# Consensys/gnark

Hardware: AMD Instinct MI355X
Metric: G1 MSM throughput, BN254, 2^24 scalar-muls on one GPU (Groth16 proofs/s at 2^24 constraints in 'groth16') (higher is better)
Workload: dtype u64 Montgomery limbs in memory; 29/28-bit limbs, v_mad_u64_u32 (32x32+64) in registers

## Files before the change

gnark_amd/csrc/msm.hip.h:

```cpp
#pragma once
#include <cstring>
#include <hipcub/hipcub.hpp>
#include <rocprim/device/device_radix_sort.hpp>

#include <string>

#include "common.hip.h"
#include "field29.hip.h"

namespace ga {

constexpr int GA_ACC29_MINW = 4;
#ifndef GA_ACC29_FP2_MINW
#define GA_ACC29_FP2_MINW 2
#endif
constexpr uint32_t MSM_SIGN = 0x80000000u;
constexpr int MSM_HOT_TASKS = 16;
constexpr uint32_t MSM_VHOT_TASKS = 512;
constexpr uint32_t MSM_VHOT_SPLIT = 64;
constexpr int MSM_GROUP = 32;

typedef rocprim::radix_sort_config<rocprim::default_config, rocprim::default_config,
                                   rocprim::radix_sort_onesweep_config<rocprim::kernel_config<1024, 21>, rocprim::kernel_config<1024, 21>, 11,
                                                                       rocprim::block_radix_rank_algorithm::match>>
// ... 661 lines not shown
__device__ __forceinline__ uint32_t msm_multi_dest(const MsmTables& mt, uint32_t dest) {
    return dest < mt.nb ? dest + blockIdx.y * mt.nb : dest + (mt.k - 1) * mt.nb + blockIdx.y * mt.max_tasks;
}

#ifdef GA_ACC29_NUM_VGPR
#define GA_ACC29_VGPR_ATTR __attribute__((amdgpu_waves_per_eu(GA_ACC29_NUM_VGPR, GA_ACC29_NUM_VGPR)))
#else
#define GA_ACC29_VGPR_ATTR
#endif
template <class F, bool COMPLETE>
__global__ void __launch_bounds__(Table29<F>::THREADS, Table29<F>::MIN_WAVES) GA_ACC29_VGPR_ATTR
msm_accumulate29_kernel(const MsmTables mt, const uint32_t* __restrict__ vals,
                        const uint32_t* __restrict__ task_start, const uint32_t* __restrict__ task_qkey_sorted,
                        const uint32_t* __restrict__ task_key_by_tid, const uint32_t* __restrict__ task_perm, uint32_t max_tasks, uint32_t seg,
                        const uint32_t* __restrict__ task_dest, XYZZ<F>* __restrict__ sums, uint32_t* __restrict__ redo_list,
                        uint32_t* __restrict__ redo_count) {
    constexpr int NW = Lazy<F>::NW;
    __shared__ uint32_t lds[4 * NW * Table29<F>::THREADS];
    uint32_t t = blockIdx.x * blockDim.x + threadIdx.x;
    if (t >= max_tasks) return;
    if (task_qkey_sorted[t] == 0xFFFFFFFFu) return;
    const uint32_t tid = task_perm[t];
    const uint32_t key = task_key_by_tid[tid];
    const uint32_t start = task_start[tid];
    LdsAcc29<F> A(lds + threadIdx.x);
    const bool have = accumulate_task29<F, COMPLETE>(A, mt.t[blockIdx.y], vals, start, start + (seg - key));
    if (!store_task29<F>(A, have, &sums[msm_multi_dest(mt, task_dest[tid])]))
        redo_list[(uint64_t)blockIdx.y * (mt.max_tasks + 2) + atomicAdd(redo_count + 2 * blockIdx.y, 1u)] = tid;
}

template <class F>
__global__ void __launch_bounds__(Table29<F>::THREADS, Table29<F>::MIN_WAVES)
msm_accumulate29_retry_kernel(const MsmTables mt, const uint32_t* __restrict__ vals,
                              const uint32_t* __restrict__ task_start, const uint32_t* __restrict__ task_key_by_tid, uint32_t seg,
                              const uint32_t* __restrict__ redo_list, const uint32_t* __restrict__ redo_count,
                              const uint32_t* __restrict__ task_dest, XYZZ<F>* __restrict__ sums, uint32_t* __restrict__ redo2_list,
                              uint32_t* __restrict__ redo2_count) {
    constexpr int NW = Lazy<F>::NW;
    __shared__ uint32_t lds[4 * NW * Table29<F>::THREADS];
    redo_list += (uint64_t)blockIdx.y * (mt.max_tasks + 2);
    redo2_list += (uint64_t)blockIdx.y * (mt.max_tasks + 2);
    const uint32_t nredo = redo_count[2 * blockIdx.y];
    LdsAcc29<F> A(lds + threadIdx.x);
    for (uint32_t r = blockIdx.x * blockDim.x + threadIdx.x; r < nredo; r += gridDim.x * blockDim.x) {
        const uint32_t tid = redo_list[r];
        const uint32_t start = task_start[tid];
        const bool have = accumulate_task29<F, true>(A, mt.t[blockIdx.y], vals, start, start + (seg - task_key_by_tid[tid]));
        if (!store_task29<F>(A, have, &sums[msm_multi_dest(mt, task_dest[tid])])) redo2_list[atomicAdd(redo2_count + 2 * blockIdx.y, 1u)] = tid;
    }
}

template <class F>
__global__ void __launch_bounds__(64)
msm_accumulate29_redo_kernel(const MsmTables mt, const uint32_t* __restrict__ vals,
                             const uint32_t* __restrict__ task_start, const uint32_t* __restrict__ task_key_by_tid,
                             uint32_t seg, const uint32_t* __restrict__ redo_list, const uint32_t* __restrict__ redo_count,
                             const uint32_t* __restrict__ task_dest, XYZZ<F>* __restrict__ sums) {
    typedef typename Lazy<F>::T T;
    redo_list += (uint64_t)blockIdx.y * (mt.max_tasks + 2);
    const uint32_t nredo = redo_count[2 * blockIdx.y];
    const uint32_t* __restrict__ table = mt.t[blockIdx.y];
    for (uint32_t r = blockIdx.x * blockDim.x + threadIdx.x; r < nredo; r += gridDim.x * blockDim.x) {
        const uint32_t tid = redo_list[r];
        const uint32_t start = task_start[tid];
        const uint32_t end = start + (seg - task_key_by_tid[tid]);
        XYZZ<F> acc = xyzz_inf<F>();
        for (uint32_t p = start; p < end; p++) {
            const uint32_t v = vals[p];
            T qx, qy;
            load_point29<F>(table, v & ~MSM_SIGN, qx, qy);
            Affine<F> q{Lazy<F>::to_mem(qx), Lazy<F>::to_mem(qy)};
            if (v & MSM_SIGN) q.y = neg(q.y);
            acc = madd(acc, q);
        }
        store_pod(&sums[msm_multi_dest(mt, task_dest[tid])], acc);
    }
}

template <class F> struct BaseFieldOf;
template <class Pp> struct BaseFieldOf<Fe<Pp>> { typedef Pp P; static constexpr bool IS_FP = true; };
template <class Pp> struct BaseFieldOf<Fe2<Pp>> { typedef Pp P; static constexpr bool IS_FP = false; };


template <class F>
__device__ __forceinline__ XYZZ<F> wave_tree_sum(XYZZ<F> acc, XYZZ<F>* sh) {
    const uint32_t lane = threadIdx.x;
    for (uint32_t stride = 32; stride >= 1; stride >>= 1) {
        sh[lane] = acc;
        __syncthreads();
        if (lane < stride) acc = add(acc, sh[lane + stride]);
        __syncthreads();
    }
    return acc;
}


template <class F>
__global__ void __launch_bounds__(64)
msm_reduce_groups_kernel(const XYZZ<F>* __restrict__ bsum, uint32_t half, uint32_t m, uint32_t groups_per_win,
                         uint32_t total_groups, XYZZ<F>* __restrict__ gsum) {
    uint32_t gid = blockIdx.x * blockDim.x + threadIdx.x;
    if (gid >= total_groups) return;
    uint32_t w = gid / groups_per_win, g = gid % groups_per_win;
    const XYZZ<F>* B = bsum + (uint64_t)w * half + (uint64_t)g * m;
    XYZZ<F> running = xyzz_inf<F>(), local = xyzz_inf<F>();
    for (int j = (int)m - 1; j >= 0; j--) {
        running = add(running, load_pod<XYZZ<F>>(&B[j]));
        local = add(local, running);
    }
    uint32_t base = g * m;
    if (base != 0) {
        XYZZ<F> r = xyzz_inf<F>();
        int top = 31 - __clz(base);
        for (int bit = top; bit >= 0; bit--) {
            r = dbl(r);
            if ((base >> bit) & 1) r = add(r, running);
        }
        local = add(local, r);
    }
    store_pod(&gsum[gid], local);
}

template <class F>
struct Lazy4 {
    typename Lazy<F>::T x, y, zz, zzz;
};
template <class F>
__device__ __forceinline__ Lazy4<F> lazy4_from_mem(const XYZZ<F>& p) {
    return {Lazy<F>::from_mem(p.x), Lazy<F>::from_mem(p.y), Lazy<F>::from_mem(p.zz), Lazy<F>::from_mem(p.zzz)};
}
template <class F>
__device__ __forceinline__ void add29(Lazy4<F>& a, const Lazy4<F>& b) {
    typedef typename Lazy<F>::T T;
    typedef typename Lazy<F>::Params P;
    constexpr int KMS = Lazy<F>::FP2 ? P::FP2Z_K : 8;
    T U1 = f29_mul(a.x, b.zz);
    T U2 = f29_mul(b.x, a.zz);
    T S1 = f29_mul(a.y, b.zzz);
    T S2 = f29_mul(b.y, a.zzz);
    T Pp = f29_sub<4>(U2, U1);
    T R = f29_sub<4>(S2, S1);
    T PP = f29_sqr(Pp);
    T PPP = f29_mul(Pp, PP);
    T Q = f29_mul(U1, PP);
    T X3 = f29_sub<4>(f29_sqr(R), f29_add(PPP, f29_add(Q, Q)));
    if constexpr (Lazy<F>::FP2) X3 = f29_partial_reduce(X3);
    a.y = f29_mul_sub<KMS>(R, f29_sub<8>(Q, X3), S1, PPP);
    a.x = X3;
    a.zz = f29_mul(f29_mul(a.zz, b.zz), PP);
    a.zzz = f29_mul(f29_mul(a.zzz, b.zzz), PPP);
}

template <class F>
__global__ void __launch_bounds__(64)
msm_reduce_groups29_kernel(const XYZZ<F>* __restrict__ bsum, uint32_t half, uint32_t m, uint32_t groups_per_win,
                           uint32_t total_groups, XYZZ<F>* __restrict__ lsum, XYZZ<F>* __restrict__ rsum,
                           uint32_t* __restrict__ redo_list, uint32_t* __restrict__ redo_count) {
    uint32_t gid = blockIdx.x * blockDim.x + threadIdx.x;
    if (gid >= total_groups) return;
    uint32_t w = gid / groups_per_win, g = gid % groups_per_win;
    const XYZZ<F>* B = bsum + (uint64_t)w * half + (uint64_t)g * m;
    Lazy4<F> running, local;
    bool r_inf = true, l_inf = true;
    for (int j = (int)m - 1; j >= 0; j--) {
        XYZZ<F> b = load_pod<XYZZ<F>>(&B[j]);
        if (!is_inf(b)) {
            Lazy4<F> lb = lazy4_from_mem<F>(b);
            if (r_inf) {
                running = lb;
                r_inf = false;
            } else {
                add29<F>(running, lb);
            }
        }
        if (!r_inf) {
            if (l_inf) {
                local = running;
                l_inf = false;
            } else {
                add29<F>(local, running);
            }
        }
    }
    XYZZ<F> lo = xyzz_inf<F>(), ro = xyzz_inf<F>();
    bool bad = false;
    if (!r_inf) {
        ro.zz = Lazy<F>::to_mem(running.zz);
        lo.zz = Lazy<F>::to_mem(local.zz);
        bad = is_zero(ro.zz) | is_zero(lo.zz);
        ro.x = Lazy<F>::to_mem(running.x);
        ro.y = Lazy<F>::to_mem(running.y);
        ro.zzz = Lazy<F>::to_mem(running.zzz);
        lo.x = Lazy<F>::to_mem(local.x);
        lo.y = Lazy<F>::to_mem(local.y);
        lo.zzz = Lazy<F>::to_mem(local.zzz);
    }
    if (bad) {
        redo_list[atomicAdd(redo_count, 1u)] = gid;
        return;
    }
    store_pod(&lsum[gid], lo);
    store_pod(&rsum[gid], ro);
}

template <class F>
__global__ void __launch_bounds__(64)
msm_reduce_groups_redo_kernel(const XYZZ<F>* __restrict__ bsum, uint32_t half, uint32_t m, uint32_t groups_per_win,
                              const uint32_t* __restrict__ redo_list, const uint32_t* __restrict__ redo_count,
                              XYZZ<F>* __restrict__ lsum, XYZZ<F>* __restrict__ rsum) {
    const uint32_t nredo = *redo_count;
    for (uint32_t r = blockIdx.x * blockDim.x + threadIdx.x; r < nredo; r += gridDim.x * blockDim.x) {
        const uint32_t gid = redo_list[r];
        uint32_t w = gid / groups_per_win, g = gid % groups_per_win;
        const XYZZ<F>* B = bsum + (uint64_t)w * half + (uint64_t)g * m;
        XYZZ<F> running = xyzz_inf<F>(), local = xyzz_inf<F>();
        for (int j = (int)m - 1; j >= 0; j--) {
            running = add(running, load_pod<XYZZ<F>>(&B[j]));
            local = add(local, running);
        }
        store_pod(&lsum[gid], local);
        store_pod(&rsum[gid], running);
    }
}

template <class F>
__device__ __forceinline__ void dbl29(Lazy4<F>& a) {
    typedef typename Lazy<F>::T T;
    typedef typename Lazy<F>::Params P;
    constexpr int KMS = Lazy<F>::FP2 ? P::FP2Z_K : 8;
    const T U = f29_add(a.y, a.y);
    const T V = f29_sqr(U);
    const T W = f29_mul(U, V);
    const T S = f29_mul(a.x, V);
    const T xx = f29_sqr(a.x);
    const T M = f29_add(f29_add(xx, xx), xx);
    T X3 = f29_sub<4>(f29_sqr(M), f29_add(S, S));
    if constexpr (Lazy<F>::FP2) X3 = f29_partial_reduce(X3);
    const T Y3 = f29_mul_sub<KMS>(M, f29_sub<8>(S, X3), W, a.y);
    a.zz = f29_mul(V, a.zz);
    a.zzz = f29_mul(W, a.zzz);
    a.x = X3;
    a.y = Y3;
}

template <class F> struct TableBatch { static constexpr int K = BaseFieldOf<F>::IS_FP ? (BaseFieldOf<F>::P::N <= 8 ? 4 : 2) : (BaseFieldOf<F>::P::N <= 8 ? 2 : 1); };

template <class F>
__global__ void __launch_bounds__(64)
msm_table29_kernel(const Affine<F>* __restrict__ bases, uint64_t n, int c, int nwin, uint32_t* __restrict__ table) {
    typedef typename Lazy<F>::T T;
    constexpr int K = TableBatch<F>::K;
    const uint64_t lanes = (uint64_t)gridDim.x * blockDim.x;
    const uint64_t gid = (uint64_t)blockIdx.x * blockDim.x + threadIdx.x;
    if (gid >= n) return;
    const T one = Lazy<F>::from_mem(FieldTraits<F>::one());
    Lazy4<F> p[K];
    bool live[K], inf[K];
#pragma unroll
    for (int q = 0; q < K; q++) {
        const uint64_t i = gid + q * lanes;
        live[q] = i < n;
        Affine<F> a = live[q] ? load_pod<Affine<F>>(&bases[i]) : Affine<F>{FieldTraits<F>::zero(), FieldTraits<F>::zero()};
        inf[q] = is_inf(a);
        p[q].x = Lazy<F>::from_mem(a.x);
        p[q].y = Lazy<F>::from_mem(a.y);
        p[q].zz = one;
        p[q].zzz = one;
    }
    for (int w = 0; w < nwin; w++) {
        if (w > 0) {
#pragma unroll
            for (int q = 0; q < K; q++)
                if (!inf[q])
                    for (int k = 0; k < c; k++) dbl29<F>(p[q]);
            T t[K], pre[K];
#pragma unroll
            for (int q = 0; q < K; q++) {
                t[q] = inf[q] ? one : f29_mul(p[q].zz, p[q].zzz);
                pre[q] = q == 0 ? t[0] : f29_mul(pre[q - 1], t[q]);
            }
            T run = f29_inv(pre[K - 1]);
#pragma unroll
            for (int q = K - 1; q >= 0; q--) {
                const T it = q > 0 ? f29_mul(run, pre[q - 1]) : run;
                if (q > 0) run = f29_mul(run, t[q]);
                if (!inf[q]) {
                    p[q].x = f29_mul(p[q].x, f29_mul(it, p[q].zzz));
                    p[q].y = f29_mul(p[q].y, f29_mul(it, p[q].zz));
                    p[q].zz = one;
                    p[q].zzz = one;
                }
            }
        }
#pragma unroll
        for (int q = 0; q < K; q++) {
            if (!live[q]) continue;
            Affine<F> h{FieldTraits<F>::zero(), FieldTraits<F>::zero()};
            if (!inf[q]) {
                h.x = f29_pack_hat(p[q].x);
                h.y = f29_pack_hat(p[q].y);
                p[q].x = Lazy<F>::unpack(h.x);
                p[q].y = Lazy<F>::unpack(h.y);
            }
            store_pod(table + ((uint64_t)w * n + gid + q * lanes) * Table29<F>::WORDS, h);
        }
    }
}

template <class F>
__global__ void __launch_bounds__(256)
msm_hat_bases_kernel(const Affine<F>* __restrict__ bases, uint64_t n, uint32_t* __restrict__ hat) {
    const uint64_t i = (uint64_t)blockIdx.x * blockDim.x + threadIdx.x;
    if (i >= n) return;
    Affine<F> a = load_pod<Affine<F>>(&bases[i]);
    if (!is_inf(a)) {
        if constexpr (BaseFieldOf<F>::IS_FP) {
            a.x = f29_hat_packed(a.x);
            a.y = f29_hat_packed(a.y);
        } else {
            a.x = {f29_hat_packed(a.x.c0), f29_hat_packed(a.x.c1)};
            a.y = {f29_hat_packed(a.y.c0), f29_hat_packed(a.y.c1)};
        }
    }
    store_pod(hat + i * Table29<F>::WORDS, a);
}

template <class F>
struct LazyPt {
    Lazy4<F> v;
    uint32_t inf;
};
template <class F>
__device__ __forceinline__ void lazy_acc(LazyPt<F>& acc, const XYZZ<F>& p) {
    if (is_inf(p)) return;
    const Lazy4<F> b = lazy4_from_mem<F>(p);
    if (acc.inf) {
        acc.v = b;
        acc.inf = 0;
    } else {
        add29<F>(acc.v, b);
    }
}
template <class F>
__device__ __forceinline__ void lazy_acc(LazyPt<F>& acc, const LazyPt<F>& b) {
    if (b.inf) return;
    if (acc.inf) acc = b;
    else add29<F>(acc.v, b.v);
}
template <class F, class Src>
__device__ __forceinline__ void block_sum29(uint32_t count, Src src, XYZZ<F>* dst, LazyPt<F>* sh, XYZZ<F>* shx, uint32_t* bad) {
    const uint32_t lane = threadIdx.x;
    LazyPt<F> acc;
    acc.inf = 1;
    for (uint32_t i = lane; i < count; i += 64) lazy_acc<F>(acc, load_pod<XYZZ<F>>(src(i)));
    for (uint32_t stride = 32; stride >= 1; stride >>= 1) {
        sh[lane] = acc;
        __syncthreads();
        if (lane < stride) lazy_acc<F>(acc, sh[lane + stride]);
        __syncthreads();
    }
    if (lane == 0) {
        XYZZ<F> out = xyzz_inf<F>();
        uint32_t b = 0;
        if (!acc.inf) {
            out.zz = Lazy<F>::to_mem(acc.v.zz);
            b = is_zero(out.zz) ? 1u : 0u;
            out.x = Lazy<F>::to_mem(acc.v.x);
            out.y = Lazy<F>::to_mem(acc.v.y);
            out.zzz = Lazy<F>::to_mem(acc.v.zzz);
        }
        if (!b) store_pod(dst, out);
        *bad = b;
    }
    __syncthreads();
    if (*bad) {
        XYZZ<F> e = xyzz_inf<F>();
        for (uint32_t i = lane; i < count; i += 64) e = add(e, load_pod<XYZZ<F>>(src(i)));
        e = wave_tree_sum(e, shx);
        if (lane == 0) store_pod(dst, e);
    }
    __syncthreads();
}

template <class F>
__global__ void __launch_bounds__(64)
msm_hot_kernel(const XYZZ<F>* __restrict__ partial, const uint32_t* __restrict__ task_off,
               const uint32_t* __restrict__ hot_list, const uint32_t* __restrict__ hot_count, XYZZ<F>* __restrict__ bsum,
               uint32_t bsum_stride, uint32_t part_stride) {
    __shared__ LazyPt<F> sh[64];
    __shared__ XYZZ<F> shx[64];
    __shared__ uint32_t bad;
    partial += (uint64_t)blockIdx.y * part_stride;
    bsum += (uint64_t)blockIdx.y * bsum_stride;
    const uint32_t nh = *hot_count;
    for (uint32_t h = blockIdx.x; h < nh; h += gridDim.x) {
        const uint32_t b = hot_list[h];
        const uint32_t t0 = task_off[b], t1 = task_off[b + 1];
        block_sum29<F>(t1 - t0, [&](uint32_t i) { return &partial[t0 + i]; }, &bsum[b], sh, shx, &bad);
    }
}

template <class F>
__global__ void __launch_bounds__(64)
msm_vhot_stage1_kernel(const XYZZ<F>* __restrict__ partial, const uint32_t* __restrict__ task_off, const uint32_t* __restrict__ vhot_list,
                       const uint32_t* __restrict__ vhot_count, XYZZ<F>* __restrict__ vtmp, uint32_t part_stride, uint32_t vtmp_stride) {
    __shared__ LazyPt<F> sh[64];
    __shared__ XYZZ<F> shx[64];
    __shared__ uint32_t bad;
    partial += (uint64_t)blockIdx.y * part_stride;
    vtmp += (uint64_t)blockIdx.y * vtmp_stride;
    const uint32_t items = *vhot_count * MSM_VHOT_SPLIT;
    for (uint32_t id = blockIdx.x; id < items; id += gridDim.x) {
        const uint32_t h = id / MSM_VHOT_SPLIT, part = id % MSM_VHOT_SPLIT;
        const uint32_t b = vhot_list[h];
        const uint32_t t0 = task_off[b], t1 = task_off[b + 1];
        const uint32_t per = (t1 - t0 + MSM_VHOT_SPLIT - 1) / MSM_VHOT_SPLIT;
        const uint32_t lo = t0 + part * per < t1 ? t0 + part * per : t1;
        const uint32_t hi = lo + per < t1 ? lo + per : t1;
        block_sum29<F>(hi - lo, [&](uint32_t i) { return &partial[lo + i]; }, &vtmp[id], sh, shx, &bad);
    }
}
template <class F>
__global__ void __launch_bounds__(64)
msm_vhot_stage2_kernel(const XYZZ<F>* __restrict__ vtmp, const uint32_t* __restrict__ vhot_list, const uint32_t* __restrict__ vhot_count,
                       XYZZ<F>* __restrict__ bsum, uint32_t bsum_stride, uint32_t vtmp_stride) {
    static_assert(MSM_VHOT_SPLIT == 64, "one partial result per lane");
    __shared__ LazyPt<F> sh[64];
    __shared__ XYZZ<F> shx[64];
    __shared__ uint32_t bad;
    vtmp += (uint64_t)blockIdx.y * vtmp_stride;
    bsum += (uint64_t)blockIdx.y * bsum_stride;
    const uint32_t nv = *vhot_count;
    for (uint32_t h = blockIdx.x; h < nv; h += gridDim.x)
        block_sum29<F>(MSM_VHOT_SPLIT, [&](uint32_t i) { return &vtmp[h * MSM_VHOT_SPLIT + i]; }, &bsum[vhot_list[h]], sh, shx, &bad);
}

template <class F>
__global__ void msm_merge_kernel(const XYZZ<F>* __restrict__ partial, const uint32_t* __restrict__ task_off, uint32_t nb,
                                 XYZZ<F>* __restrict__ bsum, uint32_t* __restrict__ hot_list, uint32_t* __restrict__ hot_count,
                                 uint32_t* __restrict__ vhot_list, uint32_t* __restrict__ vhot_count, uint32_t part_stride) {
    uint32_t b = blockIdx.x * blockDim.x + threadIdx.x;
    if (b >= nb) return;
    partial += (uint64_t)blockIdx.y * part_stride;
    bsum += (uint64_t)blockIdx.y * nb;
    uint32_t t0 = task_off[b], t1 = task_off[b + 1];
    uint32_t nt = t1 - t0;
    if (nt == 1) return;
    if (nt > MSM_VHOT_TASKS) {
        if (blockIdx.y == 0) vhot_list[atomicAdd(vhot_count, 1u)] = b;
        return;
    }
    if (nt > MSM_HOT_TASKS) {
        if (blockIdx.y == 0) hot_list[atomicAdd(hot_count, 1u)] = b;
        return;
    }
    XYZZ<F> out = xyzz_inf<F>();
    bool exact = true;
    if constexpr (BaseFieldOf<F>::P::N <= 8) {
        LazyPt<F> acc;
        acc.inf = 1;
        for (uint32_t t = t0; t < t1; t++) lazy_acc<F>(acc, load_pod<XYZZ<F>>(&partial[t]));
        exact = false;
        if (!acc.inf) {
            out.zz = Lazy<F>::to_mem(acc.v.zz);
            exact = is_zero(out.zz);
            out.x = Lazy<F>::to_mem(acc.v.x);
            out.y = Lazy<F>::to_mem(acc.v.y);
            out.zzz = Lazy<F>::to_mem(acc.v.zzz);
        }
    }
    if (exact) {
        out = xyzz_inf<F>();
        for (uint32_t t = t0; t < t1; t++) out = add(out, load_pod<XYZZ<F>>(&partial[t]));
    }
    store_pod(&bsum[b], out);
}

template <class F>
__global__ void __launch_bounds__(64)
msm_bit_partial_kernel(const XYZZ<F>* __restrict__ rsum, const XYZZ<F>* __restrict__ lsum, uint32_t groups_per_win,
                       uint32_t chunk_len, int log_chunk, XYZZ<F>* __restrict__ part) {
    __shared__ LazyPt<F> sh[64];
    __shared__ XYZZ<F> shx[64];
    __shared__ uint32_t bad;
    const uint32_t ch = blockIdx.x, b = blockIdx.y, w = blockIdx.z;
    const uint32_t nbits = gridDim.y, chunks = gridDim.x;
    const uint32_t base = ch * chunk_len;
    const XYZZ<F>* R = rsum + (uint64_t)w * groups_per_win;
    XYZZ<F>* dst = &part[((uint64_t)w * nbits + b) * chunks + ch];
    if (b == nbits - 1) {
        const XYZZ<F>* Lp = lsum + (uint64_t)w * groups_per_win;
        block_sum29<F>(chunk_len, [&](uint32_t i) { return &Lp[base + i]; }, dst, sh, shx, &bad);
    } else if ((int)b >= log_chunk) {
        block_sum29<F>(((base >> b) & 1) ? chunk_len : 0u, [&](uint32_t i) { return &R[base + i]; }, dst, sh, shx, &bad);
    } else {
        block_sum29<F>(chunk_len / 2, [&](uint32_t i) { return &R[base + (((i >> b) << (b + 1)) | (1u << b) | (i & ((1u << b) - 1)))]; }, dst, sh,
                       shx, &bad);
    }
}

template <class F>
// ... 21 lines not shown
template <class FrP>
int msm_prepare(Ctx* ctx, const void* d_scalars, size_t n, bool scalars_mont, int c, int win_lo, int win_hi, bool table,
                MsmPrepared* P, int slot = 0, int batch = 1) {
    hipStream_t st = ctx->work_stream();
    const std::string sfx = slot ? "#1" : "";
    auto key = [&](const char* k) { return std::string(k) + sfx; };
    const int nwin = FrP::BITS / c + 1;
    if (win_hi < 0) win_hi = nwin;
    if (win_lo < 0 || win_hi > nwin || win_lo >= win_hi || c < 2 || c > 24) {
        set_error("msm: bad window range [%d,%d) of %d (c=%d, table=%d)", win_lo, win_hi, nwin, c, (int)table);
        return GA_ERR_INVALID;
    }
    const int nwl = win_hi - win_lo;
    if (n == 0 || n >= (1ull << 31)) {
        set_error("msm: n=%zu outside [1, 2^31)", n);
        return GA_ERR_INVALID;
    }
    if (batch < 1 || (batch > 1 && !table)) {
        set_error("msm: a batch of scalar vectors needs a precomputed table (batch=%d, table=%d)", batch, (int)table);
        return GA_ERR_INVALID;
    }
    const uint32_t half = 1u << (c - 1);
    const uint64_t m = (uint64_t)batch * nwl * n;
    const uint64_t nb64 = table ? (uint64_t)batch * half : (uint64_t)nwl * half;
    if (m >= (1ull << 31) || nb64 >= (1ull << 31) || (table && (uint64_t)nwin * n >= (1ull << 31))) {
        set_error("msm: %d windows x %zu points exceeds the 2^31 pair index space; shard the call", nwl, n);
        return GA_ERR_INVALID;
    }
    const uint32_t nb = (uint32_t)nb64;
    uint64_t mean = m / nb + 1;
    const uint64_t min_seg = ctx->tun.msm_min_seg;
    uint64_t seg64 = mean * 4 < min_seg ? min_seg : mean * 4;
    if (nb < (1u << 19)) {
        uint64_t want = (m >> 19) + 1, lo = mean / 6 > 32 ? mean / 6 : 32;
        if (want < lo) want = lo;
        if (want < seg64) seg64 = want;
    }
    const uint32_t seg = (uint32_t)seg64;
    const uint64_t max_tasks = nb + m / seg + 1;

    uint32_t *keys, *vals, *keys2, *vals2, *off, *ntask, *task_off, *task_start, *task_key, *task_key2, *task_id, *task_perm;
    void* tmp;
    GA_CHECK(ctx->scratch_get(key("msm_vals2").c_str(), m * 4, (void**)&vals2));
    GA_CHECK(ctx->scratch_get(key("msm_off").c_str(), ((uint64_t)nb + 2) * 4, (void**)&off));
    GA_CHECK(ctx->scratch_get(key("msm_ntask").c_str(), ((uint64_t)nb + 2) * 4, (void**)&ntask));
    GA_CHECK(ctx->scratch_get(key("msm_task_off").c_str(), ((uint64_t)nb + 2) * 4, (void**)&task_off));
    GA_CHECK(ctx->scratch_get(key("msm_task_start").c_str(), max_tasks * 4, (void**)&task_start));
    GA_CHECK(ctx->scratch_get(key("msm_task_key").c_str(), max_tasks * 4, (void**)&task_key));
    GA_CHECK(ctx->scratch_get(key("msm_task_key2").c_str(), max_tasks * 4, (void**)&task_key2));
    uint32_t* task_qkey;
    GA_CHECK(ctx->scratch_get(key("msm_task_qkey").c_str(), max_tasks * 4, (void**)&task_qkey));
    GA_CHECK(ctx->scratch_get(key("msm_task_id").c_str(), max_tasks * 4, (void**)&task_id));
    GA_CHECK(ctx->scratch_get(key("msm_task_perm").c_str(), max_tasks * 4, (void**)&task_perm));
    uint32_t* task_dest;
    GA_CHECK(ctx->scratch_get(key("msm_task_dest").c_str(), max_tasks * 4, (void**)&task_dest));

    int end_bit = 1;
    while ((1ull << end_bit) <= nb64) end_bit++;
    const int xcd = ctx->tun.msm_xcd.load(std::memory_order_relaxed);
    const bool fused = msm_fused_fits(nb64) && nwl <= MSM_P1_MAXW && m >= ctx->tun.msm_fuse_min.load(std::memory_order_relaxed);
    keys = keys2 = nullptr;
    uint16_t* key_parts = nullptr;
    if (fused) {
        GA_CHECK(ctx->scratch_get("msm_keys_level1", m * 2, (void**)&key_parts));
        GA_CHECK(ctx->scratch_get("msm_vals_level1", m * 4, (void**)&vals));
    } else {
        GA_CHECK(ctx->scratch_get(key("msm_keys").c_str(), m * 4, (void**)&keys));
        GA_CHECK(ctx->scratch_get(key("msm_vals").c_str(), m * 4, (void**)&vals));
        GA_CHECK(ctx->scratch_get(key("msm_keys2").c_str(), m * 4, (void**)&keys2));
    }
    if (fused) {
        if (msm_p1_bits(nb64) == 11)
            GA_CHECK((msm_fused_sort<FrP, 11>(ctx, sfx, st, d_scalars, n, scalars_mont, c, nwin, win_lo, win_hi, table, batch, half, nb, m, key_parts, vals, vals2, off, xcd)));
        else
            GA_CHECK((msm_fused_sort<FrP, 12>(ctx, sfx, st, d_scalars, n, scalars_mont, c, nwin, win_lo, win_hi, table, batch, half, nb, m, key_parts, vals, vals2, off, xcd)));
    } else {
        {
            StageTimer tm(ctx, "msm_digits", st);
            for (int b = 0; b < batch; b++) {
                const uint32_t* sc = batch == 1 ? (const uint32_t*)d_scalars : reinterpret_cast<const uint32_t* const*>(d_scalars)[b];
                hipLaunchKernelGGL((msm_digits_kernel<FrP>), dim3((unsigned)((n + 255) / 256)), dim3(256), 0, st, sc, (uint64_t)n,
                                   scalars_mont ? 1 : 0, c, nwin, win_lo, win_hi, table ? 1 : 0, (uint32_t)b * half, (uint32_t)nb64,
                                   keys + (uint64_t)b * nwl * n, vals + (uint64_t)b * nwl * n);
            }
            GA_KERNEL_CHECK();
        }
        StageTimer tm(ctx, "msm_sort", st);
        GA_CHECK(msm_sort_pairs(ctx, key("msm_sort_tmp"), keys, keys2, vals, vals2, (size_t)m, end_bit, st));
    }
    {
        StageTimer tm(ctx, "msm_tasks", st);
        uint32_t *long_list, *long_count;
        GA_CHECK(ctx->scratch_get(key("msm_long").c_str(), (max_tasks / MSM_LONG_TASKS + 2) * 4, (void**)&long_list));
        GA_CHECK(ctx->scratch_get(key("msm_long_count").c_str(), 256, (void**)&long_count));
        int kbits = 1;
        while ((1u << kbits) <= seg) kbits++;
        const bool exact = m >= ctx->tun.msm_task_exact_min.load(std::memory_order_relaxed);
        const int qbits = exact || kbits < 7 ? kbits : 7, qshift = kbits - qbits;
        hipLaunchKernelGGL(msm_task_init_kernel, dim3((unsigned)((max_tasks + 255) / 256)), dim3(256), 0, st, task_qkey, task_id, (uint32_t)max_tasks, long_count);
        if (!fused)
            hipLaunchKernelGGL(msm_offsets_tasks_kernel, dim3((nb + 1 + 255) / 256), dim3(256), 0, st, (const uint32_t*)keys2, m, nb, seg, off, ntask);
        else
            hipLaunchKernelGGL(msm_tasks_kernel, dim3((nb + 1 + 255) / 256), dim3(256), 0, st, (const uint32_t*)off, nb, seg, ntask);
        GA_KERNEL_CHECK();
        size_t tmp_bytes = 0;
        GA_HIP_CHECK(hipcub::DeviceScan::ExclusiveSum(nullptr, tmp_bytes, ntask, task_off, (int)(nb + 1), st));
        GA_CHECK(ctx->scratch_get(key("msm_scan_tmp").c_str(), tmp_bytes + 256, &tmp));
        GA_HIP_CHECK(hipcub::DeviceScan::ExclusiveSum(tmp, tmp_bytes, ntask, task_off, (int)(nb + 1), st));
        hipLaunchKernelGGL(msm_task_list_kernel, dim3((nb + 255) / 256), dim3(256), 0, st, (const uint32_t*)off, (const uint32_t*)task_off,
                           nb, seg, qshift, task_start, task_key, task_qkey, task_dest, long_list, long_count);
        hipLaunchKernelGGL(msm_task_list_long_kernel, dim3(256), dim3(256), 0, st, (const uint32_t*)off, (const uint32_t*)task_off, nb, seg,
                           qshift, task_start, task_key, task_qkey, task_dest, (const uint32_t*)long_list, (const uint32_t*)long_count);
        GA_KERNEL_CHECK();
        size_t tb = 0;
        GA_HIP_CHECK((rocprim::radix_sort_pairs<MsmTaskSort>(nullptr, tb, task_qkey, task_key2, task_id, task_perm, (size_t)max_tasks, 0u, (unsigned)(qbits + 1), st)));
        GA_CHECK(ctx->scratch_get(key("msm_tasksort_tmp").c_str(), tb + 256, &tmp));
        GA_HIP_CHECK((rocprim::radix_sort_pairs<MsmTaskSort>(tmp, tb, task_qkey, task_key2, task_id, task_perm, (size_t)max_tasks, 0u, (unsigned)(qbits + 1), st)));
    }
    P->n = n;
    P->c = c;
    P->nwin = nwin;
    P->win_lo = win_lo;
    P->win_hi = win_hi;
    P->nsets = table ? batch : nwl;
    P->table = table;
    P->half = half;
    P->nb = nb;
    P->seg = seg;
    P->m = m;
    P->max_tasks = max_tasks;
    P->vals = vals2;
    P->task_off = task_off;
    P->task_start = task_start;
    P->task_key = task_key2;
    P->task_key_by_id = task_key;
    P->task_perm = task_perm;
    P->task_dest = task_dest;
    return GA_OK;
}


template <class F>
int msm_accumulate_reduce(Ctx* ctx, const void* d_bases, const MsmPrepared& P, XYZZ<F>* out, int horner_c = 0, const void* const* tables = nullptr,
                          int ntab = 1) {
    const uint32_t nb = P.nb, half = P.half, seg = P.seg;
    if (ntab < 1 || ntab > 4 || (ntab > 1 && (!tables || !P.table || P.nsets != 1 || horner_c != 0))) {
        set_error("msm: a multi-table pass takes 2..4 precomputed tables over one prepared scalar vector (ntab=%d, table=%d, sets=%d)", ntab, (int)P.table, P.nsets);
        return GA_ERR_INVALID;
    }
    const int nsets = ntab > 1 ? ntab : P.nsets;
    const int tuned_group = ctx->tun.msm_group.load(std::memory_order_relaxed);
    uint32_t m_groups = tuned_group ? (uint32_t)tuned_group : (uint32_t)MSM_GROUP;
    const uint64_t min_lanes = 32768;
    while (m_groups > 2 && (uint64_t)half * nsets / m_groups < min_lanes) m_groups >>= 1;
    if (m_groups > half) m_groups = half;
    const uint32_t groups_per_win = half / m_groups;
    const uint32_t total_groups = groups_per_win * nsets;
    uint32_t *hot_list, *hot_count;
    XYZZ<F>*partial, *bsum, *gsum, *gsum2, *wsum;
    GA_CHECK(ctx->scratch_get("msm_hot", ((uint64_t)nb + 2) * 4, (void**)&hot_list));
    GA_CHECK(ctx->scratch_get("msm_hot_count", 256, (void**)&hot_count));
    uint32_t* vhot_list;
    XYZZ<F>* vtmp;
    const uint64_t vhot_cap = P.max_tasks / MSM_VHOT_TASKS + 2;
    GA_CHECK(ctx->scratch_get("msm_vhot", vhot_cap * 4, (void**)&vhot_list));
    GA_CHECK(ctx->scratch_get("msm_vhot_tmp", (uint64_t)ntab * vhot_cap * MSM_VHOT_SPLIT * sizeof(XYZZ<F>), (void**)&vtmp));
    GA_CHECK(ctx->scratch_get("msm_bsum_partial", (uint64_t)ntab * ((uint64_t)nb + P.max_tasks) * sizeof(XYZZ<F>), (void**)&bsum));
    partial = bsum + (uint64_t)ntab * nb;
    const uint32_t part_stride = (uint32_t)P.max_tasks, vtmp_stride = (uint32_t)(vhot_cap * MSM_VHOT_SPLIT);
    GA_CHECK(ctx->scratch_get("msm_gsum", (uint64_t)total_groups * sizeof(XYZZ<F>), (void**)&gsum));
    GA_CHECK(ctx->scratch_get("msm_gsum2", ((uint64_t)total_groups / 1024 + 64) * sizeof(XYZZ<F>), (void**)&gsum2));
    GA_CHECK(ctx->scratch_get("msm_wsum", (uint64_t)nsets * sizeof(XYZZ<F>), (void**)&wsum));
    hipStream_t st = ctx->work_stream();
    GA_HIP_CHECK(hipMemsetAsync(hot_count, 0, 8, st));
    uint32_t h_redo_stack = 0;
    uint32_t* h_redo = ctx->pinned_words();
    if (!h_redo) h_redo = &h_redo_stack;
    *h_redo = 0;
    struct PendingRead {
        hipStream_t st;
        bool pending = false;
        ~PendingRead() {
            if (pending) hipStreamSynchronize(st);
        }
    } redo_read{ctx->work_stream()};
    const uint32_t* acc_table = (const uint32_t*)d_bases;
    {
        uint32_t *redo_list, *redo_count, *redo2_list;
        GA_CHECK(ctx->scratch_get("msm_redo", (uint64_t)ntab * (P.max_tasks + 2) * 4, (void**)&redo_list));
        GA_CHECK(ctx->scratch_get("msm_redo2", (uint64_t)ntab * (P.max_tasks + 2) * 4, (void**)&redo2_list));
        GA_CHECK(ctx->scratch_get("msm_redo_count", 256, (void**)&redo_count));
        GA_HIP_CHECK(hipMemsetAsync(redo_count, 0, 8 * ntab, st));
        StageTimer tm(ctx, "msm_accumulate");
        if (!P.table) {
            uint32_t* hat;
            GA_CHECK(ctx->scratch_get("msm_hat_bases", (uint64_t)P.n * sizeof(Affine<F>) + 256, (void**)&hat));
            hipLaunchKernelGGL((msm_hat_bases_kernel<F>), dim3((unsigned)((P.n + 255) / 256)), dim3(256), 0, st, (const Affine<F>*)d_bases,
                               (uint64_t)P.n, hat);
            acc_table = hat;
        }
        constexpr unsigned AT = Table29<F>::THREADS;
        const dim3 grid((unsigned)((P.max_tasks + AT - 1) / AT), (unsigned)ntab);
        MsmTables mt;
        mt.k = (uint32_t)ntab;
        mt.nb = nb;
        mt.max_tasks = (uint32_t)P.max_tasks;
        for (int i = 0; i < 4; i++) mt.t[i] = ntab > 1 ? (const uint32_t*)tables[i < ntab ? i : 0] : acc_table;
        if (ntab == 1 && P.table && !ctx->tun.msm_exact_redo && ctx->is_degenerate(d_bases))
            hipLaunchKernelGGL((msm_accumulate29_kernel<F, true>), grid, dim3(AT), 0, st, mt, (const uint32_t*)P.vals,
                               (const uint32_t*)P.task_start, (const uint32_t*)P.task_key, (const uint32_t*)P.task_key_by_id, (const uint32_t*)P.task_perm, (uint32_t)P.max_tasks, seg,
                               (const uint32_t*)P.task_dest, bsum, redo2_list, redo_count + 1);
        else
            hipLaunchKernelGGL((msm_accumulate29_kernel<F, false>), grid, dim3(AT), 0, st, mt, (const uint32_t*)P.vals,
                               (const uint32_t*)P.task_start, (const uint32_t*)P.task_key, (const uint32_t*)P.task_key_by_id, (const uint32_t*)P.task_perm, (uint32_t)P.max_tasks, seg,
                               (const uint32_t*)P.task_dest, bsum, redo_list, redo_count);
        if (!ctx->tun.msm_exact_redo)
            hipLaunchKernelGGL((msm_accumulate29_retry_kernel<F>), dim3(2048, (unsigned)ntab), dim3(AT), 0, st, mt, (const uint32_t*)P.vals,
                               (const uint32_t*)P.task_start, (const uint32_t*)P.task_key_by_id, seg, (const uint32_t*)redo_list,
                               (const uint32_t*)redo_count, (const uint32_t*)P.task_dest, bsum, redo2_list, redo_count + 1);
        else
            hipLaunchKernelGGL((msm_accumulate29_redo_kernel<F>), dim3(1024, (unsigned)ntab), dim3(64), 0, st, mt, (const uint32_t*)P.vals,
                               (const uint32_t*)P.task_start, (const uint32_t*)P.task_key_by_id, seg, (const uint32_t*)redo_list,
                               (const uint32_t*)redo_count, (const uint32_t*)P.task_dest, bsum);
        hipLaunchKernelGGL((msm_accumulate29_redo_kernel<F>), dim3(1024, (unsigned)ntab), dim3(64), 0, st, mt, (const uint32_t*)P.vals,
                           (const uint32_t*)P.task_start, (const uint32_t*)P.task_key_by_id, seg, (const uint32_t*)redo2_list,
                           (const uint32_t*)(redo_count + 1), (const uint32_t*)P.task_dest, bsum);
        GA_KERNEL_CHECK();
        GA_HIP_CHECK(hipMemcpyAsync(h_redo, redo_count, h_redo == &h_redo_stack ? 4 : 8 * (size_t)ntab, hipMemcpyDeviceToHost, st));
        redo_read.pending = true;
    }
    auto note_degenerate = [&]() {
        if (!P.table) return;
        if (ntab == 1) {
            if ((uint64_t)*h_redo * 4 > P.max_tasks) ctx->mark_degenerate(d_bases);
        } else if (h_redo != &h_redo_stack) {
            for (int i = 0; i < ntab; i++)
                if ((uint64_t)h_redo[2 * i] * 4 > P.max_tasks) ctx->mark_degenerate(tables[i]);
        }
    };
    {
        StageTimer tm(ctx, "msm_merge");
        const unsigned ny = (unsigned)ntab;
        hipLaunchKernelGGL((msm_merge_kernel<F>), dim3((nb + 255) / 256, ny), dim3(256), 0, st, (const XYZZ<F>*)partial,
                           (const uint32_t*)P.task_off, nb, bsum, hot_list, hot_count, vhot_list, hot_count + 1, part_stride);
        hipLaunchKernelGGL((msm_hot_kernel<F>), dim3(512, ny), dim3(64), 0, st, (const XYZZ<F>*)partial, (const uint32_t*)P.task_off,
                           (const uint32_t*)hot_list, (const uint32_t*)hot_count, bsum, nb, part_stride);
        hipLaunchKernelGGL((msm_vhot_stage1_kernel<F>), dim3(2048, ny), dim3(64), 0, st, (const XYZZ<F>*)partial, (const uint32_t*)P.task_off,
                           (const uint32_t*)vhot_list, (const uint32_t*)(hot_count + 1), vtmp, part_stride, vtmp_stride);
        hipLaunchKernelGGL((msm_vhot_stage2_kernel<F>), dim3(256, ny), dim3(64), 0, st, (const XYZZ<F>*)vtmp, (const uint32_t*)vhot_list,
                           (const uint32_t*)(hot_count + 1), bsum, nb, vtmp_stride);
        GA_KERNEL_CHECK();
    }
    const bool big_set = (uint64_t)half * nsets >= ctx->tun.reduce_lazy_min;
    const bool dense_set = P.m >= 16ull * (uint64_t)half * (uint64_t)P.nsets && !(P.table && ctx->is_sparse_set(d_bases));
    const bool lazy_reduce = big_set || dense_set;
    if (!lazy_reduce) {
        StageTimer tm(ctx, "msm_reduce");
        hipLaunchKernelGGL((msm_reduce_groups_kernel<F>), dim3((total_groups + 63) / 64), dim3(64), 0, st, (const XYZZ<F>*)bsum,
                           half, m_groups, groups_per_win, total_groups, gsum);
        const uint32_t sg = 1024;
        if (groups_per_win > 2 * sg) {
            const uint32_t nseg = groups_per_win / sg;
            hipLaunchKernelGGL((msm_segment_sum_kernel<F>), dim3(nseg * nsets), dim3(64), 0, st, (const XYZZ<F>*)gsum, sg, gsum2);
            hipLaunchKernelGGL((msm_segment_sum_kernel<F>), dim3(nsets), dim3(64), 0, st, (const XYZZ<F>*)gsum2, nseg, wsum);
        } else {
            hipLaunchKernelGGL((msm_segment_sum_kernel<F>), dim3(nsets), dim3(64), 0, st, (const XYZZ<F>*)gsum, groups_per_win, wsum);
        }
        GA_KERNEL_CHECK();
        if (horner_c > 0) {
            std::vector<XYZZ<F>> ws((size_t)nsets);
            GA_HIP_CHECK(hipMemcpyAsync(ws.data(), wsum, (size_t)nsets * sizeof(XYZZ<F>), hipMemcpyDeviceToHost, st));
            GA_HIP_CHECK(hipStreamSynchronize(st));
            note_degenerate();
            XYZZ<F> acc = xyzz_inf<F>();
            for (int w = nsets - 1; w >= 0; w--) {
                for (int k = 0; k < horner_c; k++) acc = dbl(acc);
                acc = add(acc, ws[(size_t)w]);
            }
            out[0] = acc;
            return GA_OK;
        }
        GA_HIP_CHECK(hipMemcpyAsync(out, wsum, (size_t)nsets * sizeof(XYZZ<F>), hipMemcpyDeviceToHost, st));
        GA_HIP_CHECK(hipStreamSynchronize(st));
        note_degenerate();
        return GA_OK;
    }
    int nbits = 0;
    while ((1u << nbits) < groups_per_win) nbits++;
    uint32_t sg = 1024;
    while (sg > 64 && (uint64_t)(groups_per_win / sg) * (uint64_t)(nbits + 1) * (uint64_t)nsets < 2048) sg >>= 1;
    const uint32_t chunk_len = groups_per_win > sg ? sg : groups_per_win;
    const uint32_t chunks = groups_per_win / chunk_len;
    int log_chunk = 0;
    while ((1u << log_chunk) < chunk_len) log_chunk++;
    XYZZ<F>*rsum = nullptr, *bpart = nullptr, *bits = nullptr;
    uint32_t *rg_list, *rg_count;
    GA_CHECK(ctx->scratch_get("msm_rsum", (uint64_t)total_groups * sizeof(XYZZ<F>), (void**)&rsum));
    GA_CHECK(ctx->scratch_get("msm_bpart", ((uint64_t)nsets * (nbits + 1) * chunks + 64) * sizeof(XYZZ<F>), (void**)&bpart));
    GA_CHECK(ctx->scratch_get("msm_bits", ((uint64_t)nsets * (nbits + 1) + 64) * sizeof(XYZZ<F>), (void**)&bits));
    GA_CHECK(ctx->scratch_get("msm_redo_groups", ((uint64_t)total_groups + 2) * 4, (void**)&rg_list));
    GA_CHECK(ctx->scratch_get("msm_redo_groups_count", 256, (void**)&rg_count));
    GA_HIP_CHECK(hipMemsetAsync(rg_count, 0, 4, st));
    {
        StageTimer tm(ctx, "msm_reduce");
        hipLaunchKernelGGL((msm_reduce_groups29_kernel<F>), dim3((total_groups + 63) / 64), dim3(64), 0, st, (const XYZZ<F>*)bsum,
                           half, m_groups, groups_per_win, total_groups, gsum, rsum, rg_list, rg_count);
        hipLaunchKernelGGL((msm_reduce_groups_redo_kernel<F>), dim3(256), dim3(64), 0, st, (const XYZZ<F>*)bsum, half, m_groups,
                           groups_per_win, (const uint32_t*)rg_list, (const uint32_t*)rg_count, gsum, rsum);
        hipLaunchKernelGGL((msm_bit_partial_kernel<F>), dim3(chunks, (unsigned)nbits + 1, (unsigned)nsets), dim3(64), 0, st,
                           (const XYZZ<F>*)rsum, (const XYZZ<F>*)gsum, groups_per_win, chunk_len, log_chunk, bpart);
        hipLaunchKernelGGL((msm_segment_sum29_kernel<F>), dim3((unsigned)(nsets * (nbits + 1))), dim3(64), 0, st, (const XYZZ<F>*)bpart,
                           chunks, bits);
        GA_KERNEL_CHECK();
    }
    const int rows = nbits + 1;
    std::vector<XYZZ<F>> hb((size_t)nsets * rows);
    uint32_t h_redo_groups = 0;
    GA_HIP_CHECK(hipMemcpyAsync(hb.data(), bits, (size_t)nsets * rows * sizeof(XYZZ<F>), hipMemcpyDeviceToHost, st));
    GA_HIP_CHECK(hipMemcpyAsync(&h_redo_groups, rg_count, 4, hipMemcpyDeviceToHost, st));
    GA_HIP_CHECK(hipStreamSynchronize(st));
    note_degenerate();
    if (P.table && !big_set) ctx->note_sparse_set(d_bases, (uint64_t)h_redo_groups * 4 > total_groups);
    int log_m = 0;
    while ((1u << log_m) < m_groups) log_m++;
    if (horner_c > 0) {
        const int top = horner_c * (nsets - 1) + log_m + nbits - 1;
        std::vector<std::vector<const XYZZ<F>*>> at((size_t)top + 1);
        for (int w = 0; w < nsets; w++) {
            at[(size_t)(horner_c * w)].push_back(&hb[(size_t)w * rows + nbits]);
            for (int b = 0; b < nbits; b++) at[(size_t)(horner_c * w + log_m + b)].push_back(&hb[(size_t)w * rows + b]);
        }
        XYZZ<F> acc = xyzz_inf<F>();
        for (int pos = top; pos >= 0; pos--) {
            if (pos != top) acc = dbl(acc);
            for (const XYZZ<F>* t : at[(size_t)pos]) acc = add(acc, *t);
        }
        out[0] = acc;
        return GA_OK;
    }
    for (int w = 0; w < nsets; w++) {
        XYZZ<F> acc = xyzz_inf<F>();
        for (int b = nbits - 1; b >= 0; b--) acc = add(dbl(acc), hb[(size_t)w * rows + b]);
        for (int k = 0; k < log_m; k++) acc = dbl(acc);
        out[w] = add(hb[(size_t)w * rows + nbits], acc);
    }
    return GA_OK;
}

template <class C, int G>
int msm_windows_device(Ctx* ctx, const void* d_bases, const void* d_scalars, size_t n, bool scalars_mont, int c,
                       int win_lo, int win_hi, void* h_window_sums, bool combine) {
    typedef typename GroupField<C, G>::F F;
    XYZZ<F>* out = reinterpret_cast<XYZZ<F>*>(h_window_sums);
    const int nwin = C::FrP::BITS / c + 1;
    if (win_hi < 0) win_hi = nwin;
    if (n == 0) {
        for (int w = 0; w < (combine ? 1 : win_hi - win_lo); w++) out[w] = xyzz_inf<F>();
        return GA_OK;
    }
    MsmPrepared P;
    GA_CHECK(msm_prepare<typename C::FrP>(ctx, d_scalars, n, scalars_mont, c, win_lo, win_hi, false, &P));
    return msm_accumulate_reduce<F>(ctx, d_bases, P, out, combine ? c : 0);
}

template <class C, int G>
int msm_table_device(Ctx* ctx, const void* d_table, const void* d_scalars, size_t n, bool scalars_mont, int c, void* h_sum, int win_lo,
                     int win_hi) {
    typedef typename GroupField<C, G>::F F;
    XYZZ<F>* out = reinterpret_cast<XYZZ<F>*>(h_sum);
    if (n == 0 || (win_hi >= 0 && win_hi <= win_lo)) {
        *out = xyzz_inf<F>();
        return GA_OK;
    }
    MsmPrepared P;
    GA_CHECK(msm_prepare<typename C::FrP>(ctx, d_scalars, n, scalars_mont, c, win_lo, win_hi, true, &P));
    return msm_accumulate_reduce<F>(ctx, d_table, P, out);
}

template <class C, int G>
int msm_table_device_batch(Ctx* ctx, const void* d_table, const void* const* d_scalars, int batch, size_t n, bool scalars_mont, int c,
                           void* h_sums) {
    typedef typename GroupField<C, G>::F F;
    XYZZ<F>* out = reinterpret_cast<XYZZ<F>*>(h_sums);
    if (n == 0) {
        for (int b = 0; b < batch; b++) out[b] = xyzz_inf<F>();
        return GA_OK;
    }
    MsmPrepared P;
    GA_CHECK(msm_prepare<typename C::FrP>(ctx, batch == 1 ? d_scalars[0] : (const void*)d_scalars, n, scalars_mont, c, 0, -1, true, &P, 0, batch));
    return msm_accumulate_reduce<F>(ctx, d_table, P, out);
}

template <class C, int G>
int msm_table_device_reuse(Ctx* ctx, const void* d_table, const MsmPrepared& P, void* h_sum) {
    typedef typename GroupField<C, G>::F F;
    return msm_accumulate_reduce<F>(ctx, d_table, P, reinterpret_cast<XYZZ<F>*>(h_sum));
}

template <class C, int G>
int msm_table_device_reuse_multi(Ctx* ctx, const void* const* tables, int ntab, const MsmPrepared& P, void* h_sums) {
    typedef typename GroupField<C, G>::F F;
    return msm_accumulate_reduce<F>(ctx, tables[0], P, reinterpret_cast<XYZZ<F>*>(h_sums), 0, tables, ntab);
}

template <class C>
int msm_prepare_table_scalars(Ctx* ctx, const void* d_scalars, size_t n, bool scalars_mont, int c, MsmPrepared* P, int slot, int win_lo,
                              int win_hi) {
    return msm_prepare<typename C::FrP>(ctx, d_scalars, n, scalars_mont, c, win_lo, win_hi, true, P, slot);
}

template <class C, int G>
size_t msm_table_point_bytes() {
    typedef typename GroupField<C, G>::F F;
    return Table29<F>::WORDS * 4;
}

template <class C, int G>
int msm_table_build(Ctx* ctx, const void* d_bases, size_t n, int c, void* d_table) {
    typedef typename GroupField<C, G>::F F;
    if (n == 0) return GA_OK;
    const int nwin = C::FrP::BITS / c + 1;
    StageTimer tm(ctx, "msm_table_build");
    hipLaunchKernelGGL((msm_table29_kernel<F>), dim3((unsigned)(((n + TableBatch<F>::K - 1) / TableBatch<F>::K + 63) / 64)), dim3(64), 0, ctx->work_stream(),
                       (const Affine<F>*)d_bases, (uint64_t)n, c, nwin, (uint32_t*)d_table);
    GA_KERNEL_CHECK();
    return GA_OK;
}

}
```

Measured before the change: 890.5.

## Split MSM group reduction across lane pairs with even/odd bucket interleave

The bucket-group reduction kernel now assigns two lanes per group for BN254 G1. Each lane runs a running-sum/weighted-sum over the even or odd buckets, and the halves are combined with shuffles, one doubling and extra adds. This halves the serial chain length per group and doubles the number of active lanes, at the cost of a few extra point ops and cross-lane shuffles per group. It also stops auto-shrinking the group size when the group size was explicitly tuned.

```diff
diff --git a/gnark_amd/csrc/msm.hip.h b/gnark_amd/csrc/msm.hip.h
--- a/gnark_amd/csrc/msm.hip.h
+++ b/gnark_amd/csrc/msm.hip.h
@@ -837,55 +837,110 @@
 }
 
 template <class F>
-__global__ void __launch_bounds__(64)
+__device__ void dbl29(Lazy4<F>& a);
+
+template <class F>
+struct LazyPt {
+    Lazy4<F> v;
+    uint32_t inf;
+};
+template <class F>
+__device__ __forceinline__ void lazy_acc(LazyPt<F>& acc, const XYZZ<F>& p) {
+    if (is_inf(p)) return;
+    const Lazy4<F> b = lazy4_from_mem<F>(p);
+    if (acc.inf) {
+        acc.v = b;
+        acc.inf = 0;
+    } else {
+        add29<F>(acc.v, b);
+    }
+}
+template <class F>
+__device__ __forceinline__ void lazy_acc(LazyPt<F>& acc, const LazyPt<F>& b) {
+    if (b.inf) return;
+    if (acc.inf) acc = b;
+    else add29<F>(acc.v, b.v);
+}
+template <class F> struct ReduceSplit { static constexpr int LANES = (BaseFieldOf<F>::IS_FP && BaseFieldOf<F>::P::N <= 8) ? 2 : 1; };
+
+template <class F>
+__device__ __forceinline__ LazyPt<F> pair_exchange(const LazyPt<F>& v) {
+    typedef Lazy<F> L;
+    LazyPt<F> r;
+#pragma unroll
+    for (int i = 0; i < L::NW; i++) {
+        L::set_word(r.v.x, i, __shfl_xor(L::word(v.v.x, i), 1));
+        L::set_word(r.v.y, i, __shfl_xor(L::word(v.v.y, i), 1));
+        L::set_word(r.v.zz, i, __shfl_xor(L::word(v.v.zz, i), 1));
+        L::set_word(r.v.zzz, i, __shfl_xor(L::word(v.v.zzz, i), 1));
+    }
+    r.inf = __shfl_xor(v.inf, 1);
+    return r;
+}
+
+template <class F, int SPLIT>
+__global__ void __launch_bounds__(64, SPLIT)
 msm_reduce_groups29_kernel(const XYZZ<F>* __restrict__ bsum, uint32_t half, uint32_t m, uint32_t groups_per_win,
                            uint32_t total_groups, XYZZ<F>* __restrict__ lsum, XYZZ<F>* __restrict__ rsum,
                            uint32_t* __restrict__ redo_list, uint32_t* __restrict__ redo_count) {
-    uint32_t gid = blockIdx.x * blockDim.x + threadIdx.x;
+    static_assert(SPLIT == 1 || SPLIT == 2, "one lane or a lane pair per group");
+    const uint32_t tid = blockIdx.x * blockDim.x + threadIdx.x;
+    const uint32_t gid = tid / SPLIT, h = tid % SPLIT;
     if (gid >= total_groups) return;
     uint32_t w = gid / groups_per_win, g = gid % groups_per_win;
     const XYZZ<F>* B = bsum + (uint64_t)w * half + (uint64_t)g * m;
-    Lazy4<F> running, local;
-    bool r_inf = true, l_inf = true;
-    for (int j = (int)m - 1; j >= 0; j--) {
-        XYZZ<F> b = load_pod<XYZZ<F>>(&B[j]);
-        if (!is_inf(b)) {
-            Lazy4<F> lb = lazy4_from_mem<F>(b);
-            if (r_inf) {
-                running = lb;
-                r_inf = false;
-            } else {
-                add29<F>(running, lb);
-            }
-        }
-        if (!r_inf) {
-            if (l_inf) {
-                local = running;
-                l_inf = false;
-            } else {
-                add29<F>(local, running);
-            }
-        }
-    }
-    XYZZ<F> lo = xyzz_inf<F>(), ro = xyzz_inf<F>();
-    bool bad = false;
-    if (!r_inf) {
-        ro.zz = Lazy<F>::to_mem(running.zz);
-        lo.zz = Lazy<F>::to_mem(local.zz);
-        bad = is_zero(ro.zz) | is_zero(lo.zz);
-        ro.x = Lazy<F>::to_mem(running.x);
-        ro.y = Lazy<F>::to_mem(running.y);
-        ro.zzz = Lazy<F>::to_mem(running.zzz);
-        lo.x = Lazy<F>::to_mem(local.x);
-        lo.y = Lazy<F>::to_mem(local.y);
-        lo.zzz = Lazy<F>::to_mem(local.zzz);
-    }
-    if (bad) {
-        redo_list[atomicAdd(redo_count, 1u)] = gid;
-        return;
-    }
-    store_pod(&lsum[gid], lo);
-    store_pod(&rsum[gid], ro);
+    LazyPt<F> running, local;
+    running.inf = 1;
+    local.inf = 1;
+    for (int i = (int)(m / SPLIT) - 1; i >= 0; i--) {
+        lazy_acc<F>(running, load_pod<XYZZ<F>>(&B[(uint32_t)i * SPLIT + h]));
+        if (SPLIT == 1 || h == 1 || i > 0) lazy_acc<F>(local, running);
+    }
+    if constexpr (SPLIT == 2) {
+        const LazyPt<F> other_running = pair_exchange<F>(running), other_local = pair_exchange<F>(local);
+        const LazyPt<F> r_even = running;
+        LazyPt<F> acc = h ? running : local;
+        lazy_acc<F>(acc, h ? other_running : other_local);
+        if (h == 0) {
+            if (!acc.inf) dbl29<F>(acc.v);
+            lazy_acc<F>(acc, r_even);
+        }
+        XYZZ<F> o = xyzz_inf<F>();
+        uint32_t bad = 0;
+        if (!acc.inf) {
+            o.zz = Lazy<F>::to_mem(acc.v.zz);
+            bad = is_zero(o.zz) ? 1u : 0u;
+            o.x = Lazy<F>::to_mem(acc.v.x);
+            o.y = Lazy<F>::to_mem(acc.v.y);
+            o.zzz = Lazy<F>::to_mem(acc.v.zzz);
+        }
+        bad |= __shfl_xor(bad, 1);
+        if (bad) {
+            if (h == 0) redo_list[atomicAdd(redo_count, 1u)] = gid;
+            return;
+        }
+        store_pod(h ? &rsum[gid] : &lsum[gid], o);
+    } else {
+        XYZZ<F> lo = xyzz_inf<F>(), ro = xyzz_inf<F>();
+        bool bad = false;
+        if (!running.inf) {
+            ro.zz = Lazy<F>::to_mem(running.v.zz);
+            lo.zz = Lazy<F>::to_mem(local.v.zz);
+            bad = is_zero(ro.zz) | is_zero(lo.zz);
+            ro.x = Lazy<F>::to_mem(running.v.x);
+            ro.y = Lazy<F>::to_mem(running.v.y);
+            ro.zzz = Lazy<F>::to_mem(running.v.zzz);
+            lo.x = Lazy<F>::to_mem(local.v.x);
+            lo.y = Lazy<F>::to_mem(local.v.y);
+            lo.zzz = Lazy<F>::to_mem(local.v.zzz);
+        }
+        if (bad) {
+            redo_list[atomicAdd(redo_count, 1u)] = gid;
+            return;
+        }
+        store_pod(&lsum[gid], lo);
+        store_pod(&rsum[gid], ro);
+    }
 }
 
 template <class F>
@@ -1010,28 +1065,6 @@
     store_pod(hat + i * Table29<F>::WORDS, a);
 }
 
-template <class F>
-struct LazyPt {
-    Lazy4<F> v;
-    uint32_t inf;
-};
-template <class F>
-__device__ __forceinline__ void lazy_acc(LazyPt<F>& acc, const XYZZ<F>& p) {
-    if (is_inf(p)) return;
-    const Lazy4<F> b = lazy4_from_mem<F>(p);
-    if (acc.inf) {
-        acc.v = b;
-        acc.inf = 0;
-    } else {
-        add29<F>(acc.v, b);
-    }
-}
-template <class F>
-__device__ __forceinline__ void lazy_acc(LazyPt<F>& acc, const LazyPt<F>& b) {
-    if (b.inf) return;
-    if (acc.inf) acc = b;
-    else add29<F>(acc.v, b.v);
-}
 template <class F, class Src>
 __device__ __forceinline__ void block_sum29(uint32_t count, Src src, XYZZ<F>* dst, LazyPt<F>* sh, XYZZ<F>* shx, uint32_t* bad) {
     const uint32_t lane = threadIdx.x;
@@ -1359,7 +1392,7 @@
     const int tuned_group = ctx->tun.msm_group.load(std::memory_order_relaxed);
     uint32_t m_groups = tuned_group ? (uint32_t)tuned_group : (uint32_t)MSM_GROUP;
     const uint64_t min_lanes = 32768;
-    while (m_groups > 2 && (uint64_t)half * nsets / m_groups < min_lanes) m_groups >>= 1;
+    while (!tuned_group && m_groups > 2 && (uint64_t)half * nsets / m_groups < min_lanes) m_groups >>= 1;
     if (m_groups > half) m_groups = half;
     const uint32_t groups_per_win = half / m_groups;
     const uint32_t total_groups = groups_per_win * nsets;
@@ -1510,8 +1543,12 @@
     GA_HIP_CHECK(hipMemsetAsync(rg_count, 0, 4, st));
     {
         StageTimer tm(ctx, "msm_reduce");
-        hipLaunchKernelGGL((msm_reduce_groups29_kernel<F>), dim3((total_groups + 63) / 64), dim3(64), 0, st, (const XYZZ<F>*)bsum,
-                           half, m_groups, groups_per_win, total_groups, gsum, rsum, rg_list, rg_count);
+        if (ReduceSplit<F>::LANES == 2 && m_groups % 2 == 0)
+            hipLaunchKernelGGL((msm_reduce_groups29_kernel<F, ReduceSplit<F>::LANES>), dim3((unsigned)(((uint64_t)total_groups * 2 + 63) / 64)),
+                               dim3(64), 0, st, (const XYZZ<F>*)bsum, half, m_groups, groups_per_win, total_groups, gsum, rsum, rg_list, rg_count);
+        else
+            hipLaunchKernelGGL((msm_reduce_groups29_kernel<F, 1>), dim3((total_groups + 63) / 64), dim3(64), 0, st, (const XYZZ<F>*)bsum,
+                               half, m_groups, groups_per_win, total_groups, gsum, rsum, rg_list, rg_count);
         hipLaunchKernelGGL((msm_reduce_groups_redo_kernel<F>), dim3(256), dim3(64), 0, st, (const XYZZ<F>*)bsum, half, m_groups,
                            groups_per_win, (const uint32_t*)rg_list, (const uint32_t*)rg_count, gsum, rsum);
         hipLaunchKernelGGL((msm_bit_partial_kernel<F>), dim3(chunks, (unsigned)nbits + 1, (unsigned)nsets), dim3(64), 0, st,
```

After: 899.5 (median of 3 runs). No clear change (+1.0%).
